# microsoft/OpenMSFTL

Measured on AMD Instinct MI355X. Metric: device-resident grad encode+decode GB/s at 1/2/4/8 MI355X; % HBM roofline, higher is better.
Workload: dtype fp32; 1 GPU; BASELINE configs[3] per-GPU shard: clients x 134,217,728-fp32 gradients, top-k f=0.1 encode -> FedAVG decode-accumulate; clients_per_gpu=128, n=134217728, codec=top, k=13421773, parallelism=dp1

## Files before the change

### openmsftl_amd/csrc/fc_capi.hip

```cpp
#include <math.h>
#include <stdarg.h>
#include <stdio.h>
#include <stdlib.h>
#include <string.h>

#include <algorithm>
#include <mutex>
#include <vector>

#include <hip/hip_ext.h>

#include "fc_state.h"

using namespace fc;

static thread_local char g_err[512];

static int fail(int code, const char* fmt, ...) {
  va_list ap;
  va_start(ap, fmt);
  vsnprintf(g_err, sizeof g_err, fmt, ap);
  va_end(ap);
  return code;
}

#define FC_CHECK(cond, ...) \
  do { if (!(cond)) return fail(FC_ERR_ARG, __VA_ARGS__); } while (0)
#define FC_LAUNCHED(name)                                                          \
  do {                                                                             \
    hipError_t e_ = hipGetLastError();                                             \
    if (e_ != hipSuccess) return fail(FC_ERR_HIP, "%s: %s", name, hipGetErrorString(e_)); \
  } while (0)

static uint32_t index_bits(uint64_t n) {
  uint32_t b = 1;
  while (b < 32 && (1ull << b) < n) ++b;
  return b;
}

static uint32_t num_chunks(uint64_t n) { return (uint32_t)((n + kChunk - 1) / kChunk); }

static WsPtrs ws_ptrs(void* ws, uint64_t n) {
  const WsLayout L = WsLayout::of(n);
  char* b = static_cast<char*>(ws);
  WsPtrs W;
  W.st = reinterpret_cast<TopkState*>(b);
  W.hist1 = reinterpret_cast<uint32_t*>(b + L.off_hist1);
  W.tick = reinterpret_cast<uint32_t*>(b + L.off_tick);
  W.ehist = reinterpret_cast<uint32_t*>(b + L.off_ehist);
  W.chist = reinterpret_cast<uint32_t*>(b + L.off_chist);
  W.small = reinterpret_cast<uint64_t*>(b + L.off_small);
  W.smallv = reinterpret_cast<uint32_t*>(b + L.off_smallv);
  W.pub = reinterpret_cast<uint32_t*>(b + L.off_pub);
  W.ccnt = reinterpret_cast<uint32_t*>(b + L.off_status);
  W.cand = reinterpret_cast<uint64_t*>(b + L.off_cand);
  W.cand_cap = L.cand_cap;
  return W;
}

static uint32_t decode_grid(uint64_t n, uint32_t per_cu = kDecBlocksPerCU) {
#ifdef FC_DEBUG_BUILD
  static const uint32_t forced = [] {
    const char* e = getenv("FC_DECODE_GRID");
    return e ? (uint32_t)atoi(e) : 0u;
  }();
#else
  constexpr uint32_t forced = 0;
#endif
  uint32_t g = forced ? forced : 256u * per_cu;
  const uint32_t nch = num_chunks(n);
  return g < nch ? g : nch;
}

constexpr int FC_MAX_SAMPLE_SEGS = 1024;
constexpr int FC_SAMPLE_DIV = 64;
constexpr int FC_SAMPLE_DIV_SINGLE = 32;
constexpr int FC_MAX_SAMPLE_SEGS_SINGLE = 2048;
constexpr int FC_SAMPLE_ROUNDS = 4;
constexpr int FC_CAND_PER_BIN = 128;
static uint32_t cand_bins_log2(uint64_t n, const SamplePlan& P) {
  if (P.full || P.lo_all || P.hi_none) return 12;
  const double S = (double)P.nseg * 1024.0;
  const double expect = (double)(P.r_lo - P.r_hi) * (double)n / S;
  uint32_t lg = 8;
  while (lg < 12 && (double)(1u << lg) * FC_CAND_PER_BIN < expect) ++lg;
  return lg;
}
static SamplePlan make_plan(uint64_t n, uint64_t k, bool single = false) {
  SamplePlan P;
  memset(&P, 0, sizeof P);
  P.n = n;
  if (n <= kFullSampleMax) {
    P.full = 1;
    P.nseg = (uint32_t)((n + 1023) / 1024);
    P.r_hi = P.r_lo = (int64_t)k;
  } else {
    uint64_t seg = n / (single ? FC_SAMPLE_DIV_SINGLE : FC_SAMPLE_DIV) / 1024;
    if (seg < 64) seg = 64;
    const uint64_t cap = single ? FC_MAX_SAMPLE_SEGS_SINGLE : FC_MAX_SAMPLE_SEGS;
    if (seg > cap) seg = cap;
    P.nseg = (uint32_t)seg;
    const double S = (double)seg * 1024.0;
    const double q = (double)k / (double)n;
    const double rho = q * S;
    const double m = 6.0 * sqrt(S * q * (1.0 - q)) + 16.0;
    P.r_hi = (int64_t)floor(rho - m);
    P.r_lo = (int64_t)ceil(rho + m);
    if (P.r_lo > (int64_t)S) P.lo_all = 1;
  }
  if (P.r_hi < 1) P.hi_none = 1;
  P.cbins_log2 = 12;
  P.segs = n <= (32ull << 20) ? 2u : (uint32_t)kSampleSegs;
  P.pstride = (P.nseg + P.segs - 1) / P.segs;
  P.np = 0;
  while (P.np < P.segs && P.np * P.pstride < P.nseg) ++P.np;
  double Sp = 0.0;
  for (uint32_t j = 0; j < P.np; ++j) {
    const uint64_t st = seg_start(P, pilot_seg(P, j));
    const uint64_t lim = P.full ? std::min<uint64_t>(st + 1024, n) : st + 1024;
    Sp += (double)(lim - st);
  }
  const double S = P.full ? (double)n : (double)P.nseg * 1024.0;
  const double q = (double)k / (double)n;
  const double sig = sqrt(Sp * q * (1.0 - q));
  const int64_t isp = (int64_t)Sp;
  P.pr_hi = std::max<int64_t>(1, (int64_t)floor((double)P.r_hi * Sp / S - 7.0 * sig - 8.0));
  P.pr_lo = std::min<int64_t>(isp, (int64_t)ceil((double)P.r_lo * Sp / S + 7.0 * sig + 8.0));
  if (P.pr_hi > isp) P.pr_hi = isp;
  if (P.pr_lo < P.pr_hi) P.pr_lo = P.pr_hi;
  return P;
}

static int check_common(const float* g, uint64_t n, void* ws, size_t ws_bytes) {
  FC_CHECK(g != nullptr, "g is NULL");
  FC_CHECK(n >= 1 && n <= 0xffffffffull, "n=%llu outside [1, 2^32-1]", (unsigned long long)n);
  FC_CHECK(((uintptr_t)g & 15) == 0, "g must be 16-byte aligned");
  FC_CHECK(ws != nullptr, "workspace is NULL");
  if (ws_bytes < WsLayout::of(n).bytes)
    return fail(FC_ERR_WORKSPACE, "workspace %zu B < %llu B needed", ws_bytes,
// ... 903 lines not shown
```

### openmsftl_amd/csrc/fc_decode.hip

```cpp
#include <type_traits>

#include "fc_state.h"

namespace fc {

struct PktCache {
  const void* idx;
  const float* val;
  const uint32_t* bitmap;
  const uint32_t* cnt;
  uint64_t thresh, seed, offset;
  double p;
  uint32_t ib, codec, key_mode;
  float w;
};

__device__ __forceinline__ PktCache load_pkt(const fc_packet_view& v) {
  PktCache c;
  c.idx = v.idx; c.val = v.val; c.bitmap = v.bitmap; c.cnt = v.cnt; c.w = v.weight;
  const fc_packet_hdr* h = v.hdr;
  c.thresh = h->thresh; c.seed = h->seed; c.offset = h->offset; c.p = h->p;
  c.ib = h->index_bits; c.codec = h->codec; c.key_mode = h->key_mode;
  return c;
}
// ... 449 lines not shown
          const float s2 = __fadd_rn(tile[loc], term);
          tile[loc] = s2;
          if (poison) cntC[loc] = (uint8_t)(cntC[loc] + 1u);
        } else {
          tile[loc] = v;
        }
      };
      if (!generic) {
        uint32_t loc[kSR];
        bool ok[kSR];
        float tv[kSR];
#pragma unroll
        for (int r = 0; r < kSR; ++r) {
          const uint32_t e = (uint32_t)(tid + r * kSBlock);
          loc[r] = ids[d][r];
          const bool keep = thresh == 0 || comp_of(mag_key(vs[d][r]), (uint32_t)base + loc[r], ib) >= thresh;
          ok[r] = e < cn[d] && keep && loc[r] < (uint32_t)kChunk;
          tv[r] = 0.f;
          if (ACC && ok[r]) tv[r] = tile[loc[r]];
        }
#pragma unroll
        for (int r = 0; r < kSR; ++r) {
          if (!ok[r]) continue;
          if (ACC) {
            const float s2 = __fadd_rn(tv[r], __fmul_rn(vs[d][r], w));
            tile[loc[r]] = s2;
            if (poison) cntC[loc[r]] = (uint8_t)(cntC[loc[r]] + 1u);
          } else {
            tile[loc[r]] = vs[d][r];
          }
        }
      } else {
        const PktCache pk = meta_pkt_s(pm);
        for (int r = 0; r < kSR; ++r) {
          const uint32_t e = (uint32_t)(tid + r * kSBlock);
          const uint32_t lc = ids[d][r];
          const float v = vs[d][r];
          if (e < cn[d] && entry_kept(pk, (uint32_t)base + lc, v)) fold(lc, scale ? (float)((double)v / pk.p) : v);
        }
      }
      if (cn[d] > (uint32_t)(kSR * kSBlock)) {
        const PktCache pk = meta_pkt_s(pm);
        gf32* pval = (gf32*)uni_ptr(pm.val) + base;
        gu16* pidx = (gu16*)uni_ptr(pm.idx) + base;
        for (uint32_t e = (uint32_t)(kSR * kSBlock + tid); e < cn[d]; e += kSBlock) {
          const uint32_t lc = pidx[e];
          const float v = pval[e];
          if (entry_kept(pk, (uint32_t)base + lc, v)) fold(lc, scale ? (float)((double)v / pk.p) : v);
        }
        __builtin_amdgcn_s_waitcnt(0x0F70);
      }
      __syncthreads();
      if (m + 1 == M) {
        write_tile(c);
        const uint32_t cnext = c + G;
        if (t + 1 < T) {
          __syncthreads();
          init_tile(cnext);
          __syncthreads();
        }
      }
    }
  };
  issue_cnt(0);
  issue_cnt(1);
  issue_ent(0);
  init_tile(blockIdx.x);
  __syncthreads();
  for (uint32_t t0 = 0; t0 < T; t0 += 2 * kSGroup) {
    issue_cnt(0);
    issue_ent(1);
    process(0, t0);
    if (t0 + kSGroup >= T) break;
    issue_cnt(1);
    issue_ent(0);
    process(1, t0 + kSGroup);
  }
}

constexpr int kQBlock = 256;
constexpr int kQuarter = kChunk / 4;
constexpr int FC_QR = 4;
constexpr int kQR = FC_QR;
constexpr int FC_QG = 3;
constexpr int kQGroup = FC_QG;
constexpr int FC_QTAIL = 8;
constexpr int kQTail = FC_QTAIL > FC_QR ? FC_QTAIL : FC_QR;

static_assert(kSparseMaxM <= 128, "k_fold_q reads the quarter offsets of <= 128 packets "
                                   "(lanes 0..63 and 64..127)");

struct QMeta {
  const void* idx;
  const float* val;
  const void* qoff;
  const fc_packet_hdr* hdr;
  uint64_t thresh;
  float w;
  uint32_t flags;
};
constexpr uint32_t kQNoQoff = 1u << 25;
constexpr uint64_t kQWhole = 1ull << 63;

template <bool DEC>
__device__ __forceinline__ void fold_q_entry(const PktCache& pk, float w, float* qt,
                                             uint32_t qbase, uint32_t id, float v) {
  if (!entry_kept(pk, id, v)) return;
  const float x = pk.codec == FC_CODEC_DROPOUT_UNBIASED ? (float)((double)v / pk.p) : v;
  const uint32_t loc = id - qbase;
  if (loc < (uint32_t)kQuarter) qt[loc] = DEC ? x : __fadd_rn(qt[loc], __fmul_rn(x, w));
}

template <bool ACC_IN, bool DEC = false>
__global__ __launch_bounds__(kQBlock, 4) void k_fold_q(DecodeArgs a) {
  __shared__ __attribute__((aligned(16))) float tile[kChunk];
  __shared__ QMeta s_meta[kSparseMaxM];
  __shared__ uint32_t s_mark[4][kQuarter / 32];
  __shared__ uint32_t s_slow;
  const int tid = threadIdx.x, lane = lane_id();
  const int q = __builtin_amdgcn_readfirstlane(tid >> 6);
  const uint32_t M = (uint32_t)a.m;
  const uint32_t c = blockIdx.x;
  const uint64_t base = (uint64_t)c * kChunk;
  const uint32_t qbase = (uint32_t)base + (uint32_t)(q * kQuarter);
  if (tid == 0) s_slow = 0;
  s_mark[q][lane] = 0u;
  __syncthreads();
  if (tid < (int)M) {
    const fc_packet_view v = DEC ? a.one : a.views[tid];
    const fc_packet_hdr* h = v.hdr;
    QMeta d;
    d.idx = v.idx; d.val = v.val; d.hdr = h;
    d.qoff = v.qoff ? (const void*)v.qoff : (const void*)v.cnt;
    d.thresh = h->thresh; d.w = v.weight;
    const uint32_t codec = h->codec, key_mode = h->key_mode;
    const float dz = (codec == FC_CODEC_DROPOUT_UNBIASED && h->p == 0.0) ? __uint_as_float(0x7fc00000u) : 0.0f;
    const bool poison = __fmul_rn(dz, v.weight) != __fmul_rn(dz, v.weight);
    const bool generic = codec == FC_CODEC_DROPOUT_UNBIASED || (key_mode == FC_KEY_PHILOX && d.thresh != 0) ||
                         (d.thresh >> (h->index_bits & 0xffu)) >= 0x7f800000ull;
    d.flags = (h->index_bits & 0xffu) | ((codec & 0xffu) << 8) | ((key_mode & 0xffu) << 16) |
              ((uint32_t)poison << 24) | (v.qoff ? 0u : kQNoQoff);
    s_meta[tid] = d;
    if (poison || generic) atomicOr(&s_slow, 1u);
  }
  __syncthreads();
  const bool slow = s_slow != 0;
  typedef __attribute__((address_space(1))) const uint64_t gu64;
  typedef __attribute__((address_space(1))) const uint32_t gu32c;
  auto qload = [&](uint32_t m) -> uint64_t {
    const QMeta& pm = s_meta[m];
    if (pm.flags & kQNoQoff) return kQWhole | ((gu32c*)pm.qoff)[c];
    return ((gu64*)pm.qoff)[c];
  };
  const uint64_t qo0 = (uint32_t)lane < M ? qload((uint32_t)lane) : 0ull;
  const uint64_t qo1 = (uint32_t)lane + 64 < M ? qload((uint32_t)lane + 64) : 0ull;
  auto qcount = [&](uint64_t v) -> uint32_t {
    if (v & kQWhole) return kQuarter + 1u;
    const uint32_t st = q == 0 ? 0u : (uint32_t)(v >> (16 * (q - 1))) & 0xffffu;
    const uint32_t en = q == 3 ? (uint32_t)(v >> 48) : (uint32_t)(v >> (16 * q)) & 0xffffu;
    return en - st;
  };
  const bool dense_q = __any(qcount(qo0) > (uint32_t)(kQTail * 64) || qcount(qo1) > (uint32_t)(kQTail * 64));
  auto range = [&](uint32_t m, uint32_t& st, uint32_t& en) {
    const uint64_t src = m < 64 ? qo0 : qo1;
    const uint32_t lo = (uint32_t)__builtin_amdgcn_readlane((int)(uint32_t)src, (int)(m & 63));
    const uint32_t hi = (uint32_t)__builtin_amdgcn_readlane((int)(uint32_t)(src >> 32), (int)(m & 63));
    const uint64_t v = ((uint64_t)hi << 32) | lo;
    st = q == 0 ? 0u : (uint32_t)(v >> (16 * (q - 1))) & 0xffffu;
    en = q == 3 ? (uint32_t)(v >> 48) : (uint32_t)(v >> (16 * q)) & 0xffffu;
    if (v & kQWhole) { st = 0u; en = lo & 0xffffu; }
  };
  float* qt = tile + q * kQuarter;
  float dz0 = 0.f;
  if (DEC) {
    const fc_packet_hdr* h = (const fc_packet_hdr*)uni_ptr(s_meta[0].hdr);
    if (h->codec == FC_CODEC_DROPOUT_UNBIASED && h->p == 0.0) dz0 = __uint_as_float(0x7fc00000u);
  }
#pragma unroll
  for (int i = 0; i < kQuarter / 256; ++i) {
    const uint32_t loc = (uint32_t)(i * 256 + lane * 4);
    float4 v = make_float4(dz0, dz0, dz0, dz0);
    if (ACC_IN) v = load4(reinterpret_cast<const float*>(a.out), (uint64_t)qbase + loc, a.n);
    *reinterpret_cast<float4*>(&qt[loc]) = v;
  }
  if (slow || dense_q) {
    for (uint32_t m = 0; m < M; ++m) {
      uint32_t st, en;
      range(m, st, en);
      const QMeta& pm = s_meta[m];
      const fc_packet_hdr* h = (const fc_packet_hdr*)uni_ptr(pm.hdr);
      PktCache pk;
      pk.thresh = uni64(pm.thresh); pk.ib = uni32(pm.flags) & 0xffu;
      pk.codec = (uni32(pm.flags) >> 8) & 0xffu; pk.key_mode = (uni32(pm.flags) >> 16) & 0xffu;
      pk.seed = h->seed; pk.offset = h->offset; pk.p = h->p;
      const float w = __uint_as_float(uni32(__float_as_uint(pm.w)));
      gu16* pidx = (gu16*)uni_ptr(pm.idx) + base;
      gf32* pval = (gf32*)uni_ptr(pm.val) + base;
      if (!DEC && ((uni32(pm.flags) >> 24) & 1u)) {
        for (uint32_t e = st + lane; e < en; e += 64) {
          const uint32_t id = (uint32_t)base + pidx[e];
          const uint32_t loc = id - qbase;
          if (loc < (uint32_t)kQuarter && entry_kept(pk, id, pval[e]))
            atomicOr(&s_mark[q][loc >> 5], 1u << (loc & 31));
        }
        const uint32_t bits = s_mark[q][lane];
        for (int b = 0; b < 32; ++b)
          if (!((bits >> b) & 1u)) qt[lane * 32 + b] = __uint_as_float(0x7fc00000u);
        s_mark[q][lane] = 0u;
      }
      for (uint32_t e = st + lane; e < en; e += 64)
        fold_q_entry<DEC>(pk, w, qt, qbase, (uint32_t)base + pidx[e], pval[e]);
    }
  } else {
    uint32_t ids_[2][kQGroup][kQR];
    float vs_[2][kQGroup][kQR];
    uint32_t qn_[2][kQGroup];
    auto issue = [&](int sl, uint32_t m0) {
#pragma unroll
      for (int d = 0; d < kQGroup; ++d) {
        const uint32_t m = min(m0 + (uint32_t)d, M - 1);
        uint32_t st, en;
        range(m, st, en);
        qn_[sl][d] = en - st;
        const QMeta& pm = s_meta[m];
        gf32* val = (gf32*)uni_ptr(pm.val) + base + st;
        gu16* idx = (gu16*)uni_ptr(pm.idx) + base + st;
        const uint32_t last = en > st ? en - st - 1u : 0u;
#pragma unroll
        for (int r = 0; r < kQR; ++r) {
          const uint32_t e = min((uint32_t)(lane + r * 64), last);
          vs_[sl][d][r] = val[e];
          ids_[sl][d][r] = idx[e];
        }
      }
    };
    auto process = [&](int sl, uint32_t m0) {
#pragma unroll
      for (int d = 0; d < kQGroup; ++d) {
        const uint32_t m = m0 + (uint32_t)d;
        if (m >= M) break;
        const QMeta& pm = s_meta[m];
        const float w = __uint_as_float(uni32(__float_as_uint(pm.w)));
        const uint64_t thresh = uni64(pm.thresh);
        const uint32_t ib = uni32(pm.flags) & 0xffu;
        const float Tf = __uint_as_float((uint32_t)(thresh >> ib));
        const uint32_t Ti = (uint32_t)(thresh & ((1ull << ib) - 1ull));
        const uint32_t b32 = (uint32_t)base;
        const uint32_t Tr = Ti <= b32 ? 0u : min(Ti - b32, (uint32_t)kChunk);
        const uint32_t qn = qn_[sl][d];
        const int lim = (int)qn - lane;
        float* slot[kQR];
        float tv[kQR];
        float* dummy = reinterpret_cast<float*>(&s_mark[q][lane]);
#pragma unroll
        for (int r = 0; r < kQR; ++r) {
          const uint32_t lc = ids_[sl][d][r];
          const float v = vs_[sl][d][r];
          const float av = __builtin_fabsf(v);
          const bool ok = (lim > r * 64) & (!(av <= Tf) | ((av == Tf) & (lc >= Tr)));
          slot[r] = ok ? qt + (lc & (uint32_t)(kQuarter - 1)) : dummy;
          tv[r] = DEC ? 0.f : *slot[r];
        }
#pragma unroll
        for (int r = 0; r < kQR; ++r)
          *slot[r] = DEC ? vs_[sl][d][r] : __fadd_rn(tv[r], __fmul_rn(vs_[sl][d][r], w));
        if (kQTail > kQR && qn > (uint32_t)(kQR * 64)) {
          uint32_t st, en;
          range(m, st, en);
          gf32* val = (gf32*)uni_ptr(pm.val) + base;
          gu16* idx = (gu16*)uni_ptr(pm.idx) + base;
          for (uint32_t e = st + (uint32_t)(kQR * 64) + lane; e < en; e += 64) {
            const uint32_t lc = idx[e];
            const float v = val[e];
            const float av = __builtin_fabsf(v);
            const uint32_t l2 = lc & (uint32_t)(kQuarter - 1);
            if (!(av <= Tf) | ((av == Tf) & (lc >= Tr)))
              qt[l2] = DEC ? v : __fadd_rn(qt[l2], __fmul_rn(v, w));
          }
        }
      }
    };
    issue(0, 0);
    for (uint32_t m0 = 0; m0 < M; m0 += 2 * kQGroup) {
      issue(1, m0 + kQGroup);
      process(0, m0);
      if (m0 + kQGroup >= M) break;
      issue(0, m0 + 2 * kQGroup);
      process(1, m0 + kQGroup);
    }
  }
  float* out = reinterpret_cast<float*>(a.out);
#pragma unroll
  for (int i = 0; i < kQuarter / 256; ++i) {
    const uint32_t loc = (uint32_t)(i * 256 + lane * 4);
    store_out(out, (uint64_t)qbase + loc, a.n, *reinterpret_cast<const float4*>(&qt[loc]));
  }
}

struct DecResArgs {
  const uint16_t* idx;
  const float* val;
  const uint64_t* qoff;
  fc_packet_hdr* hdr;
  float* out;
  uint64_t n;
  uint32_t ib, pad_;
  WsPtrs W;
};

__global__ __launch_bounds__(kQBlock, 4) void k_decode_res(DecResArgs a) {
  __shared__ __attribute__((aligned(16))) float tile[kChunk];
  __shared__ uint32_t s_skip[4][kQuarter / 32];
  __shared__ uint32_t s_fin[4];
  __shared__ uint64_t s_T;
  const int tid = threadIdx.x, lane = lane_id();
  const int q = __builtin_amdgcn_readfirstlane(tid >> 6);
  const uint32_t c = blockIdx.x;
  const uint64_t base = (uint64_t)c * kChunk;
  const uint32_t qbase = (uint32_t)base + (uint32_t)(q * kQuarter);
  const uint64_t qo = a.qoff[c];
  TopkState* S = a.W.st;
  const uint32_t t_lo = S->t_lo, t_hi = S->t_hi, sbin = S->sbin;
  const uint32_t beta = S->rb_beta, flags = S->rb_flags, cnt = S->rb_cnt;
  const bool gather = (flags & 3u) == 0;
  float* qt = tile + q * kQuarter;
#pragma unroll
  for (int i = 0; i < kQuarter / 256; ++i)
    *reinterpret_cast<float4*>(&qt[i * 256 + lane * 4]) = make_float4(0.f, 0.f, 0.f, 0.f);
  s_skip[q][lane] = 0u;
  if (lane == 0) s_fin[q] = 0u;
  __builtin_amdgcn_fence(__ATOMIC_RELEASE, "wavefront");
  __builtin_amdgcn_wave_barrier();
  bool finisher = false;
  if (!(flags & 1u)) {
    const uint32_t st = q == 0 ? 0u : (uint32_t)(qo >> (16 * (q - 1))) & 0xffffu;
    const uint32_t en = q == 3 ? (uint32_t)(qo >> 48) : (uint32_t)(qo >> (16 * q)) & 0xffffu;
    gu16* pidx = (gu16*)a.idx + base;
    gf32* pval = (gf32*)a.val + base;
    for (uint32_t e = st + (uint32_t)lane; e < en; e += 64) {
      const uint32_t lc = pidx[e];
      const float v = pval[e];
      const uint32_t key = mag_key(v);
      const uint32_t loc = lc & (uint32_t)(kQuarter - 1);
      const uint32_t bin = (key - t_lo) >> sbin;
      const bool cand = key <= t_hi;
      if (!cand || bin > beta) {
        qt[loc] = v;
      } else if (bin == beta && gather) {
        const uint32_t pos = atomicAdd(&S->small_n, 1u);
        st_agent(&a.W.small[pos], comp_of(key, (uint32_t)base + lc, a.ib));
        st_agent(&a.W.smallv[pos], __float_as_uint(v));
        atomicOr(&s_skip[q][loc >> 5], 1u << (loc & 31));
        asm volatile("s_waitcnt vmcnt(0)" ::: "memory");
        if (atomicAdd(&S->small_done, 1u) == cnt - 1u) finisher = true;
      }
    }
  }
  if (finisher) s_fin[q] = 1u;
  __builtin_amdgcn_fence(__ATOMIC_ACQ_REL, "wavefront");
  __builtin_amdgcn_wave_barrier();
  float* out = a.out;
#pragma unroll
  for (int i = 0; i < kQuarter / 256; ++i) {
    const uint32_t loc = (uint32_t)(i * 256 + lane * 4);
    const float4 v = *reinterpret_cast<const float4*>(&qt[loc]);
    const uint32_t skip = (s_skip[q][loc >> 5] >> (loc & 31)) & 0xfu;
    const uint64_t e = (uint64_t)qbase + loc;
    if (!skip) {
      store_out(out, e, a.n, v);
    } else {
      if (!(skip & 1u) && e + 0 < a.n) out[e + 0] = v.x;
// ... 129 lines not shown
```

### openmsftl_amd/csrc/fc_state.h

```cpp
#pragma once
#include <stdint.h>
#include "../../include/fedcodec.h"
#include "fc_common.h"

namespace fc {

struct alignas(16) TopkState {
  uint64_t ticket;
  uint64_t L64;
  uint64_t e_prefix;
  uint32_t err;
  uint32_t a_done, b_done, r_done;
  uint32_t pad0_[3];
  uint32_t win_flag;
  uint32_t pad1_[2];
  uint32_t t_lo, t_hi;
  uint32_t sbin;
  uint32_t cand_on, n_cand, cand_over, ent_over;
  uint32_t small_n;
  uint32_t e_shift, e_rank, e_matched, e_done, e_ticket, e_status;
  uint32_t gen;
  uint32_t small_done;
  uint32_t fz_seq;
  uint32_t hgen;
  uint32_t rb_beta, rb_rin, rb_cnt;
  uint32_t rb_flags;
  uint32_t rb_nent, rb_ncand;
  uint32_t shard_ent[kShards];
  uint32_t shard_cnd[kShards];
};
static_assert(sizeof(TopkState) <= 1024, "state block");

constexpr int FC_SAMPLE_SHARDS = 2;
constexpr int FC_CAND_SHARDS = 2;
constexpr int kSampleShards = FC_SAMPLE_SHARDS;
constexpr int kCandShards = FC_CAND_SHARDS;
constexpr int kTickGroups = 16;
constexpr int kTickStride = 64;
constexpr int kTickWords = (kTickGroups + 1) * kTickStride;
constexpr int kPubCopies = 64;
constexpr int kWinCopies = 16;
constexpr int kPubStride = 32;
constexpr int kPubWords = (kPubCopies + kWinCopies) * kPubStride;

struct WsLayout {
  uint64_t nchunks, cand_cap;
  uint64_t off_hist1, off_tick, off_ehist, off_chist, off_small, off_smallv, off_pub, off_status,
      off_cand, bytes;
  __host__ __device__ static WsLayout of(uint64_t n) {
    WsLayout L;
    L.nchunks = (n + kChunk - 1) / kChunk;
    L.cand_cap = L.nchunks * kCandSlot;
    uint64_t o = 1024;
    L.off_hist1 = o;  o += 4ull * kHistBins * kSampleShards;
    L.off_tick = o;   o += 4ull * kTickWords * 3;
    L.off_ehist = o;  o += 4ull * kHistBins;
    o += 8192;
    L.off_chist = o;  o += 4ull * kHistBins * kCandShards;
    L.off_small = o;  o += 8ull * kSmallCap;
    L.off_smallv = o; o += 4ull * kSmallCap;
    L.off_pub = o;    o += 4ull * kPubWords;
    L.off_status = o; o += 4ull * (L.nchunks ? L.nchunks : 1);
    o = (o + 15) & ~15ull;
    L.off_cand = o;   o += 8ull * L.cand_cap;
    L.bytes = (o + 255) & ~255ull;
    return L;
  }
};

struct HdrInit {
  uint64_t seed, offset;
  double p;
  uint32_t n, k, ib, codec, format, key_mode;
};

struct WsPtrs {
  TopkState* st;
  uint32_t *hist1, *tick, *ehist, *chist;
  uint64_t* small;
  uint32_t* smallv;
  uint32_t* pub;
  uint32_t* ccnt;
  uint64_t* cand;
  uint64_t cand_cap;
};

__device__ __forceinline__ WsPtrs ws_shift(WsPtrs W, uint64_t bytes) {
  W.st = reinterpret_cast<TopkState*>(reinterpret_cast<char*>(W.st) + bytes);
  W.hist1 = reinterpret_cast<uint32_t*>(reinterpret_cast<char*>(W.hist1) + bytes);
  W.tick = reinterpret_cast<uint32_t*>(reinterpret_cast<char*>(W.tick) + bytes);
  W.ehist = reinterpret_cast<uint32_t*>(reinterpret_cast<char*>(W.ehist) + bytes);
  W.chist = reinterpret_cast<uint32_t*>(reinterpret_cast<char*>(W.chist) + bytes);
  W.small = reinterpret_cast<uint64_t*>(reinterpret_cast<char*>(W.small) + bytes);
  W.smallv = reinterpret_cast<uint32_t*>(reinterpret_cast<char*>(W.smallv) + bytes);
  W.pub = reinterpret_cast<uint32_t*>(reinterpret_cast<char*>(W.pub) + bytes);
  W.ccnt = reinterpret_cast<uint32_t*>(reinterpret_cast<char*>(W.ccnt) + bytes);
  W.cand = reinterpret_cast<uint64_t*>(reinterpret_cast<char*>(W.cand) + bytes);
  return W;
}

__device__ __forceinline__ void write_hdr_static(fc_packet_hdr* h, const HdrInit& hi) {
  h->thresh = 0; h->lower = 0;
  h->n = hi.n; h->k = hi.k; h->n_entries = 0; h->index_bits = hi.ib;
  h->codec = hi.codec; h->status = FC_STATUS_OK; h->n_definite = 0; h->n_cand = 0;
  h->seed = hi.seed; h->offset = hi.offset; h->p = hi.p;
  h->chunk = kChunk; h->format = hi.format; h->key_mode = hi.key_mode;
  h->reserved[0] = h->reserved[1] = h->reserved[2] = 0;
}

struct SamplePlan {
  uint64_t n;
  uint32_t nseg;
  uint32_t full;
  int64_t r_hi, r_lo;
  uint32_t hi_none, lo_all;
  uint32_t np;
  uint32_t pstride;
  int64_t pr_hi, pr_lo;
  uint32_t cbins_log2;
  uint32_t segs;
};
constexpr int FC_SAMPLE_SEGS_PER_WG = 4;
constexpr int kPilotSegs = FC_SAMPLE_SEGS_PER_WG;
constexpr uint64_t kFullSampleMax = 1ull << 20;

__host__ __device__ __forceinline__ uint64_t seg_start(const SamplePlan& P, uint32_t s) {
  if (P.full || P.nseg == 1) return (uint64_t)s * 1024;
  return ((uint64_t)s * (P.n - 1024) / (P.nseg - 1)) & ~3ull;
}
__host__ __device__ __forceinline__ uint32_t pilot_seg(const SamplePlan& P, uint32_t j) {
  return j * P.pstride;
}

}
```

### openmsftl_amd/csrc/fc_topk.hip

```cpp
#include <type_traits>

#include "fc_state.h"

namespace fc {

template <int KM>
__device__ __forceinline__ uint4 keys4(const float4& x, uint64_t e, uint64_t seed,
                                       uint64_t off) {
  if (KM == kKeyMag) return make_uint4(mag_key(x.x), mag_key(x.y), mag_key(x.z), mag_key(x.w));
  return make_uint4(philox_word(e, seed, off) >> 1, philox_word(e + 1, seed, off) >> 1,
                    philox_word(e + 2, seed, off) >> 1, philox_word(e + 3, seed, off) >> 1);
}
template <int KM>
__device__ __forceinline__ uint32_t key1(float x, uint64_t i, uint64_t seed, uint64_t off) {
  if (KM == kKeyMag) return mag_key(x);
  return philox_word(i, seed, off) >> 1;
}
__device__ __forceinline__ uint32_t u4get(const uint4& v, int j) {
  return j == 0 ? v.x : j == 1 ? v.y : j == 2 ? v.z : v.w;
}

__device__ __forceinline__ void rank_owner(uint32_t r, uint32_t excl, uint32_t sum, uint32_t total,
                                           uint32_t* s_own) {
  if (r >= 1 && r <= total && r > excl && r <= excl + sum) { s_own[0] = threadIdx.x; s_own[1] = excl; }
// ... 860 lines not shown
  MagShared m;
};

template <bool DENSE, int NW>
__device__ __forceinline__ void fused_mag_wg(const CompactArgs& a0, const SamplePlan& P,
                                             const HdrInit& HI, uint32_t nsamp) {
  __shared__ __attribute__((aligned(16))) FusedShared u;
  __shared__ MagState s_st;
  TopkState* S = a0.W.st;
  const uint32_t pub = sload2(&S->fz_seq).x + 1u;
  if (blockIdx.x < nsamp) {
    if (threadIdx.x >= kBlock) return;
    sample_body<kKeyMag, false>(a0.g, P, 0ull, 0ull, a0.W, a0.ib, a0.hdr, HI, blockIdx.x, nsamp, false, u.s, pub);
    return;
  }
  const uint32_t chunk = blockIdx.x - nsamp;
  float x[MagGeo<NW>::kQ];
  if (chunk < 1024u) __builtin_amdgcn_s_sleep(90);
  const uint32_t* rec = &a0.W.pub[(blockIdx.x % kPubCopies) * kPubStride];
  const uint32_t tag = pub | 0x80000000u;
  typedef __attribute__((address_space(4))) const fc_rec4 fc_crec4;
  const bool try_s = !DENSE && chunk >= (uint32_t)FC_FUSED_SREC;
  fc_rec4 sr = {0u, 0u, 0u, 0u};
  if (try_s) sr = *(fc_crec4*)rec;
  mag_load<NW>(a0.g, chunk, a0.n, x);
  FC_TR(24);
  MagState st;
  if (try_s && sr.w == tag) {
    st.t_lo = sr.x; st.t_hi = sr.y; st.sbin = sr.z; st.cand_on = 1u;
    st.L64 = (uint64_t)sr.x << a0.ib;
  } else {
  if (threadIdx.x == 0) {
    uint32_t it = 0;
    fc_rec4 r = ld16_agent(rec);
    while (r.w != tag && ++it < kSpinMax) {
      __builtin_amdgcn_s_sleep(4);
      r = ld16_agent(rec);
    }
    if (it >= kSpinMax) st_agent(&S->err, 1u);
    MagState m;
    m.t_lo = r.x; m.t_hi = r.y; m.sbin = r.z; m.cand_on = 1u;
    m.L64 = (uint64_t)r.x << a0.ib;
    s_st = m;
  }
  __syncthreads();
  FC_TR(25);
  st = s_st;
  }
  compact_mag_item<NW, MagShared, DENSE, true, !DENSE>(a0, mag_out(a0, 0u), chunk, st, x, u.m);
  FC_TR(26);
}
template <bool DENSE>
__global__ __launch_bounds__(kCBlock, FC_MAG1_WAVES_PER_EU) void k_fused_mag(CompactArgs a0, SamplePlan P,
                                                                              HdrInit HI, uint32_t nsamp) {
  fused_mag_wg<DENSE, 8>(a0, P, HI, nsamp);
}
template __global__ void k_fused_mag<false>(CompactArgs, SamplePlan, HdrInit, uint32_t);
template __global__ void k_fused_mag<true>(CompactArgs, SamplePlan, HdrInit, uint32_t);

struct ResolveArgs {
  uint32_t ib, nchunks;
  uint64_t k;
  const uint16_t* idx;
  const float* val;
  const uint32_t* cnt;
  uint64_t seed, offset;
  uint32_t key_mode;
  fc_packet_hdr* hdr;
  WsPtrs W;
  const fc_encode_job* jobs;
  uint64_t ws_stride;
  float* dense;
  uint32_t rbin;
};

constexpr int kResolveChunksMax = 1024;

template <bool BIN>
__global__ __launch_bounds__(kBlock) void k_resolve(ResolveArgs a0) {
  ResolveArgs a = a0;
  apply_job(a);
  __shared__ uint64_t sv[kSmallCap];
  __shared__ uint32_t s_pre[kResolveChunksMax];
  __shared__ uint32_t s_tmp[8], s_out[4], s_flag, s_cnt, s_base, s_tot[2];
  __shared__ uint64_t s_T;
  uint32_t* h = reinterpret_cast<uint32_t*>(sv);
  TopkState* S = a.W.st;
  const int tid = threadIdx.x;
  FC_TR(8);
  uint32_t se = 0, sc = 0;
  if (tid < kShards) { se = S->shard_ent[tid]; sc = S->shard_cnd[tid]; }
  const uint32_t t_lo = S->t_lo, t_hi = S->t_hi, sbin = S->sbin, err = S->err;
  const bool rbin = a.rbin != 0;
  const uint32_t per = (a.nchunks + gridDim.x - 1) / gridDim.x;
  const uint32_t c0 = blockIdx.x * per;
  const uint32_t c1 = min(c0 + per, a.nchunks);
  const uint32_t nc = c1 > c0 ? c1 - c0 : 0u;
  const uint32_t cc_early = (nc <= (uint32_t)kBlock && (uint32_t)tid < nc) ? a.W.ccnt[c0 + tid] : 0u;
  uint32_t hv[kHistBins / kBlock];
  const bool own_hist = !BIN && !rbin;
#pragma unroll
  for (int j = 0; j < kHistBins / kBlock; ++j) hv[j] = own_hist ? a.W.chist[j * kBlock + tid] : 0u;
  static_assert(kShards == 64, "shard totals: one wave");
  if (tid < 64) {
    se = wave_sum(se);
    sc = wave_sum(sc);
    if (tid == 0) {
      s_tot[0] = se; s_tot[1] = sc;
      if (!BIN && rbin) { s_out[0] = ld_agent(&S->rb_beta); s_out[1] = ld_agent(&S->rb_rin);
                          s_out[2] = ld_agent(&S->rb_cnt); }
    }
  }
#pragma unroll
  for (int j = 0; j < kHistBins / kBlock; ++j) h[j * kBlock + tid] = hv[j];
  __syncthreads();
  const uint32_t n_ent = s_tot[0], n_cand = s_tot[1];
  const uint32_t n_hi = n_ent - n_cand;
  const bool bad = err || n_cand > n_ent || (uint64_t)n_ent < a.k || (uint64_t)n_hi > a.k;
  const uint32_t rank = bad ? 0u : (uint32_t)(a.k - n_hi);
  bool retry = bad || per > (uint32_t)kResolveChunksMax;
  uint32_t beta = 0, r_in = 1, cnt_beta = 0;
  if (!BIN && !retry && rank > 0) {
    if (own_hist) {
      find_rank_desc(h, rank, s_tmp, s_out);
      beta = s_out[0]; r_in = s_out[1]; cnt_beta = h[beta];
    } else {
      beta = s_out[0]; r_in = s_out[1]; cnt_beta = s_out[2];
    }
    retry = cnt_beta > (uint32_t)kSmallCap || cnt_beta < r_in;
    __syncthreads();
  }
  const bool binning = BIN && !retry && rank > 0;
  const bool walk = BIN ? binning : (!retry && (rank > 0 || a.dense));
  if (BIN && !binning) return;
  if (walk) {
    for (uint32_t lc = tid; lc < nc; lc += kBlock) {
      const uint32_t c = c0 + lc;
      const uint32_t cc = nc <= (uint32_t)kBlock ? cc_early : a.W.ccnt[c];
      s_pre[lc] = cc > (uint32_t)kCandSlot ? (a.cnt[c] | 0x80000000u) : cc;
    }
    __syncthreads();
  }
  FC_TR(10);
  constexpr int kGatherU = 8;
  uint32_t tpc = 64;
  while (tpc > 4 && tpc * nc > (uint32_t)kBlock) tpc >>= 1;
  uint64_t v0[kGatherU];
#pragma unroll
  for (int u = 0; u < kGatherU; ++u) v0[u] = ~0ull;
  auto for_cands = [&](bool reuse, auto&& fn) {
    const uint32_t cpr = (uint32_t)kBlock / tpc;
    for (uint32_t cb = 0; cb < nc; cb += cpr) {
      const uint32_t lc = cb + (uint32_t)tid / tpc, q = (uint32_t)tid % tpc;
      const uint32_t info = lc < nc ? s_pre[lc] : 0u;
      const uint32_t sz = info & 0x7fffffffu;
      const bool ovf = (info >> 31) != 0;
      const uint32_t c = c0 + lc;
      for (uint32_t r0 = q; r0 < sz; r0 += tpc * kGatherU) {
        const bool first = cb == 0 && r0 == q;
        uint64_t v[kGatherU];
#pragma unroll
        for (int u = 0; u < kGatherU; ++u) {
          const uint32_t r = r0 + (uint32_t)u * tpc;
          v[u] = ~0ull;
          if (reuse && first) {
            v[u] = v0[u];
          } else if (r < sz) {
            if (!ovf) {
              v[u] = a.W.cand[(uint64_t)c * kCandSlot + r];
            } else {
              const uint64_t p = (uint64_t)c * kChunk + r;
              const uint32_t id = c * (uint32_t)kChunk + a.idx[p];
              const uint32_t key = a.key_mode == FC_KEY_PHILOX ? (philox_word(id, a.seed, a.offset) >> 1)
                                                               : mag_key(a.val[p]);
              v[u] = (key >= t_lo && key <= t_hi) ? comp_of(key, id, a.ib) : ~0ull;
            }
          }
        }
        if (first && !reuse) {
#pragma unroll
          for (int u = 0; u < kGatherU; ++u) v0[u] = v[u];
        }
        fn(v);
      }
    }
  };
  auto bin_of = [&](uint64_t v) { return (((uint32_t)(v >> a.ib)) - t_lo) >> sbin; };
  if constexpr (BIN) {
    for_cands(false, [&](const uint64_t (&v)[kGatherU]) {
#pragma unroll
      for (int u = 0; u < kGatherU; ++u)
        if (v[u] != ~0ull) atomicAdd(&h[bin_of(v[u])], 1u);
    });
    __syncthreads();
    FC_TR(29);
    const uint32_t nb = min((uint32_t)kHistBins, ((t_hi - t_lo) >> sbin) + 1u);
    flush_hist(a.W.chist + (blockIdx.x % kCandShards) * kHistBins, h, nb);
    FC_TR(27);
    if (!last_block_arrive_tree(a.W.tick + 2 * kTickWords, gridDim.x, blockIdx.x, &s_flag)) return;
    constexpr int kPer = kHistBins / kBlock;
    uint32_t t[kPer];
#pragma unroll
    for (int j = 0; j < kPer; ++j) t[j] = 0;
#pragma unroll
    for (int sh = 0; sh < kCandShards; ++sh)
#pragma unroll
      for (int j = 0; j < kPer; ++j)
        if ((uint32_t)(j * kBlock + tid) < nb) t[j] += ld_agent(&a.W.chist[sh * kHistBins + j * kBlock + tid]);
#pragma unroll
    for (int j = 0; j < kPer; ++j) h[j * kBlock + tid] = t[j];
    __syncthreads();
    find_rank_desc(h, rank, s_tmp, s_out);
    if (tid == 0) {
      st_agent(&S->rb_beta, s_out[0]); st_agent(&S->rb_rin, s_out[1]);
      st_agent(&S->rb_cnt, h[s_out[0]]);
    }
    for (int sh = 0; sh < kCandShards; ++sh)
      for (uint32_t b = tid; b < nb; b += kBlock) a.W.chist[sh * kHistBins + b] = 0u;
    FC_TR(28);
    return;
  } else {
    if (!retry && rank > 0) {
      if (tid == 0) s_cnt = 0;
      __syncthreads();
      for_cands(false, [&](const uint64_t (&v)[kGatherU]) {
#pragma unroll
        for (int u = 0; u < kGatherU; ++u) {
          if (v[u] != ~0ull && bin_of(v[u]) == beta) {
            const uint32_t q = atomicAdd(&s_cnt, 1u);
            if (q < (uint32_t)kSmallCap) sv[q] = v[u];
          }
        }
      });
      __syncthreads();
      if (tid == 0 && s_cnt) s_base = atomicAdd(&S->small_n, min(s_cnt, (uint32_t)kSmallCap));
      __syncthreads();
      const uint32_t mine = min(s_cnt, (uint32_t)kSmallCap);
      for (uint32_t q = tid; q < mine; q += kBlock)
        if (s_base + q < (uint32_t)kSmallCap) st_agent(&a.W.small[s_base + q], sv[q]);
    }
    FC_TR(11);
    const uint64_t imask = (1ull << a.ib) - 1;
    if (a.dense && walk) {
      const uint32_t below = rank > 0 ? beta : 0xffffffffu;
      for_cands(rank > 0, [&](const uint64_t (&v)[kGatherU]) {
#pragma unroll
        for (int u = 0; u < kGatherU; ++u)
          if (v[u] != ~0ull && bin_of(v[u]) < below) a.dense[v[u] & imask] = 0.0f;
      });
    }
    if (!last_block_arrive_tree(a.W.tick + kTickWords, gridDim.x, blockIdx.x, &s_flag, 16)) return;
    FC_TR(12);
    uint64_t T = 0;
    uint32_t first_below = 0, list_n = 0;
    bool sorted = false;
    if (retry) {
      T = 0;
    } else if (a.k == 0) {
      T = kSelectNothing;
    } else if (rank == 0) {
      T = ((uint64_t)t_hi + 1) << a.ib;
    } else if (cnt_beta <= (uint32_t)kBlock) {
      uint64_t mine = 0;
      if ((uint32_t)tid < cnt_beta) { mine = ld_agent(&a.W.small[tid]); sv[tid] = mine; }
      __syncthreads();
      if ((uint32_t)tid < cnt_beta) {
        uint32_t larger = 0;
        for (uint32_t j = 0; j < cnt_beta; ++j) larger += sv[j] > mine ? 1u : 0u;
        if (larger == r_in - 1) s_T = mine;
      }
      __syncthreads();
      T = s_T;
      list_n = cnt_beta;
    } else {
      uint32_t P2 = 1;
      while (P2 < cnt_beta) P2 <<= 1;
      for (uint32_t i = tid; i < P2; i += kBlock) sv[i] = i < cnt_beta ? ld_agent(&a.W.small[i]) : 0ull;
      __syncthreads();
      bitonic_desc(sv, P2);
      T = sv[r_in - 1];
      first_below = r_in; list_n = cnt_beta; sorted = true;
    }
    const bool other_err = ld_agent(&S->err) != 0u;
    const uint32_t status = retry || other_err ? (uint32_t)FC_STATUS_RETRY_EXACT : (uint32_t)FC_STATUS_OK;
    FC_TR(14);
    if (a.dense && status == FC_STATUS_OK && rank > 0) {
      for (uint32_t i = (sorted ? first_below : 0u) + tid; i < list_n; i += kBlock) {
        const uint64_t v = sv[i];
        if (v < T) a.dense[v & imask] = 0.0f;
      }
    }
    if (!rbin)
      for (int b = tid; b < kHistBins; b += kBlock) a.W.chist[b] = 0;
    if (tid == 0) {
      a.hdr->thresh = T;
      a.hdr->n_entries = n_ent;
      if (status != FC_STATUS_OK) a.hdr->status = status;
      a.hdr->n_definite = n_hi;
      a.hdr->n_cand = n_cand;
      S->small_n = 0; S->err = 0;
      S->fz_seq += 1u;
    }
    FC_TR(15);
  }
}
template __global__ void k_resolve<true>(ResolveArgs);
template __global__ void k_resolve<false>(ResolveArgs);

__global__ __launch_bounds__(kBlock) void k_beta(ResolveArgs a) {
  __shared__ uint32_t h[kHistBins];
  __shared__ uint32_t s_tmp[8], s_out[4], s_tot[2];
  beta_body<false>(a.W, a.k, h, s_tmp, s_out, s_tot);
  TopkState* S = a.W.st;
  const int tid = threadIdx.x;
  for (int b = tid; b < kHistBins; b += kBlock) a.W.chist[b] = 0;
  if (tid == 0) {
    const uint32_t flags = S->rb_flags, n_ent = S->rb_nent, n_cand = S->rb_ncand;
    a.hdr->n_entries = n_ent;
    a.hdr->n_definite = n_ent - n_cand;
    a.hdr->n_cand = n_cand;
    if (flags & 1u) { a.hdr->thresh = 0; a.hdr->status = FC_STATUS_RETRY_EXACT; }
    else if (flags & 2u) a.hdr->thresh = ((uint64_t)S->t_hi + 1) << a.ib;
    S->err = 0;
    S->small_n = 0; S->small_done = 0;
    S->fz_seq += 1u;
  }
}


struct EngineArgs {
  const float* g;
  uint64_t n;
// ... 119 lines not shown
```

Measured before the change: 4307 GB/s.

## Record per-chunk bin occupancy to skip chunks in sparse resolve; deepen fold pipeline

During the binning pass, each chunk now records a 64-bit occupancy mask of which histogram bin groups its candidates hit. The sparse resolve pass uses that mask to compact the chunk list to only those chunks that can hold the target bin, which skips gathering from chunks that cannot contribute. The decode fold kernel also replaces its two-slot, three-packet-group double buffer with a six-slot ring of single-packet groups to keep more loads in flight. The cost is extra workspace, a shuffle reduction per chunk, shared-memory atomics for compaction, and more registers in the fold ring.

```diff
diff --git a/openmsftl_amd/csrc/fc_capi.hip b/openmsftl_amd/csrc/fc_capi.hip
--- a/openmsftl_amd/csrc/fc_capi.hip
+++ b/openmsftl_amd/csrc/fc_capi.hip
@@ -55,6 +55,7 @@
   W.ccnt = reinterpret_cast<uint32_t*>(b + L.off_status);
   W.cand = reinterpret_cast<uint64_t*>(b + L.off_cand);
   W.cand_cap = L.cand_cap;
+  W.occ = reinterpret_cast<uint64_t*>(b + L.off_occ);
   return W;
 }
 
diff --git a/openmsftl_amd/csrc/fc_decode.hip b/openmsftl_amd/csrc/fc_decode.hip
--- a/openmsftl_amd/csrc/fc_decode.hip
+++ b/openmsftl_amd/csrc/fc_decode.hip
@@ -555,8 +555,12 @@
 constexpr int kQuarter = kChunk / 4;
 constexpr int FC_QR = 4;
 constexpr int kQR = FC_QR;
-constexpr int FC_QG = 3;
+constexpr int FC_QG = 1;
 constexpr int kQGroup = FC_QG;
+constexpr int FC_QSLOTS = 6;
+constexpr int kQSlots = FC_QSLOTS;
+static_assert(kQSlots >= 2, "k_fold_q: one slot folds while the others load");
+static_assert(kQSlots * kQGroup * 2 * FC_QR <= 63, "k_fold_q: the ring's loads must fit vmcnt");
 constexpr int FC_QTAIL = 8;
 constexpr int kQTail = FC_QTAIL > FC_QR ? FC_QTAIL : FC_QR;
 
@@ -685,9 +689,9 @@
         fold_q_entry<DEC>(pk, w, qt, qbase, (uint32_t)base + pidx[e], pval[e]);
     }
   } else {
-    uint32_t ids_[2][kQGroup][kQR];
-    float vs_[2][kQGroup][kQR];
-    uint32_t qn_[2][kQGroup];
+    uint32_t ids_[kQSlots][kQGroup][kQR];
+    float vs_[kQSlots][kQGroup][kQR];
+    uint32_t qn_[kQSlots][kQGroup];
     auto issue = [&](int sl, uint32_t m0) {
 #pragma unroll
       for (int d = 0; d < kQGroup; ++d) {
@@ -753,13 +757,15 @@
         }
       }
     };
-    issue(0, 0);
-    for (uint32_t m0 = 0; m0 < M; m0 += 2 * kQGroup) {
-      issue(1, m0 + kQGroup);
-      process(0, m0);
-      if (m0 + kQGroup >= M) break;
-      issue(0, m0 + 2 * kQGroup);
-      process(1, m0 + kQGroup);
+#pragma unroll
+    for (int s = 0; s < kQSlots - 1; ++s) issue(s, (uint32_t)(s * kQGroup));
+    for (uint32_t m0 = 0; m0 < M; m0 += kQSlots * kQGroup) {
+#pragma unroll
+      for (int s = 0; s < kQSlots; ++s) {
+        if (s > 0 && m0 + (uint32_t)(s * kQGroup) >= M) break;
+        issue((s + kQSlots - 1) % kQSlots, m0 + (uint32_t)((s + kQSlots - 1) * kQGroup));
+        process(s, m0 + (uint32_t)(s * kQGroup));
+      }
     }
   }
   float* out = reinterpret_cast<float*>(a.out);
diff --git a/openmsftl_amd/csrc/fc_state.h b/openmsftl_amd/csrc/fc_state.h
--- a/openmsftl_amd/csrc/fc_state.h
+++ b/openmsftl_amd/csrc/fc_state.h
@@ -46,7 +46,7 @@
 struct WsLayout {
   uint64_t nchunks, cand_cap;
   uint64_t off_hist1, off_tick, off_ehist, off_chist, off_small, off_smallv, off_pub, off_status,
-      off_cand, bytes;
+      off_cand, off_occ, bytes;
   __host__ __device__ static WsLayout of(uint64_t n) {
     WsLayout L;
     L.nchunks = (n + kChunk - 1) / kChunk;
@@ -63,6 +63,7 @@
     L.off_status = o; o += 4ull * (L.nchunks ? L.nchunks : 1);
     o = (o + 15) & ~15ull;
     L.off_cand = o;   o += 8ull * L.cand_cap;
+    L.off_occ = o;    o += 8ull * (L.nchunks ? L.nchunks : 1);
     L.bytes = (o + 255) & ~255ull;
     return L;
   }
@@ -83,6 +84,7 @@
   uint32_t* ccnt;
   uint64_t* cand;
   uint64_t cand_cap;
+  uint64_t* occ;
 };
 
 __device__ __forceinline__ WsPtrs ws_shift(WsPtrs W, uint64_t bytes) {
@@ -96,6 +98,7 @@
   W.pub = reinterpret_cast<uint32_t*>(reinterpret_cast<char*>(W.pub) + bytes);
   W.ccnt = reinterpret_cast<uint32_t*>(reinterpret_cast<char*>(W.ccnt) + bytes);
   W.cand = reinterpret_cast<uint64_t*>(reinterpret_cast<char*>(W.cand) + bytes);
+  W.occ = reinterpret_cast<uint64_t*>(reinterpret_cast<char*>(W.occ) + bytes);
   return W;
 }
 
diff --git a/openmsftl_amd/csrc/fc_topk.hip b/openmsftl_amd/csrc/fc_topk.hip
--- a/openmsftl_amd/csrc/fc_topk.hip
+++ b/openmsftl_amd/csrc/fc_topk.hip
@@ -966,7 +966,7 @@
   apply_job(a);
   __shared__ uint64_t sv[kSmallCap];
   __shared__ uint32_t s_pre[kResolveChunksMax];
-  __shared__ uint32_t s_tmp[8], s_out[4], s_flag, s_cnt, s_base, s_tot[2];
+  __shared__ uint32_t s_tmp[8], s_out[4], s_flag, s_cnt, s_base, s_tot[2], s_nl;
   __shared__ uint64_t s_T;
   uint32_t* h = reinterpret_cast<uint32_t*>(sv);
   TopkState* S = a.W.st;
@@ -990,7 +990,7 @@
     se = wave_sum(se);
     sc = wave_sum(sc);
     if (tid == 0) {
-      s_tot[0] = se; s_tot[1] = sc;
+      s_tot[0] = se; s_tot[1] = sc; s_nl = 0;
       if (!BIN && rbin) { s_out[0] = ld_agent(&S->rb_beta); s_out[1] = ld_agent(&S->rb_rin);
                           s_out[2] = ld_agent(&S->rb_cnt); }
     }
@@ -1017,29 +1017,36 @@
   const bool binning = BIN && !retry && rank > 0;
   const bool walk = BIN ? binning : (!retry && (rank > 0 || a.dense));
   if (BIN && !binning) return;
+  static_assert(kResolveChunksMax <= 1024 && kChunk < (1 << 14), "s_pre word");
+  const bool sparse = !BIN && rbin && !a.dense && walk;
+  uint32_t nl = nc;
   if (walk) {
     for (uint32_t lc = tid; lc < nc; lc += kBlock) {
       const uint32_t c = c0 + lc;
+      const uint64_t occ = sparse ? a.W.occ[c] : ~0ull;
       const uint32_t cc = nc <= (uint32_t)kBlock ? cc_early : a.W.ccnt[c];
-      s_pre[lc] = cc > (uint32_t)kCandSlot ? (a.cnt[c] | 0x80000000u) : cc;
+      const uint32_t word = (cc > (uint32_t)kCandSlot ? (a.cnt[c] | 0x80000000u) : cc) | (lc << 14);
+      if (!sparse) s_pre[lc] = word;
+      else if ((occ >> (beta >> 6)) & 1ull) s_pre[atomicAdd(&s_nl, 1u)] = word;
     }
     __syncthreads();
+    if (sparse) nl = s_nl;
   }
   FC_TR(10);
   constexpr int kGatherU = 8;
   uint32_t tpc = 64;
-  while (tpc > 4 && tpc * nc > (uint32_t)kBlock) tpc >>= 1;
+  while (tpc > 4 && tpc * nl > (uint32_t)kBlock) tpc >>= 1;
   uint64_t v0[kGatherU];
 #pragma unroll
   for (int u = 0; u < kGatherU; ++u) v0[u] = ~0ull;
-  auto for_cands = [&](bool reuse, auto&& fn) {
+  auto for_cands = [&](bool reuse, auto&& fn, auto&& done) {
     const uint32_t cpr = (uint32_t)kBlock / tpc;
-    for (uint32_t cb = 0; cb < nc; cb += cpr) {
-      const uint32_t lc = cb + (uint32_t)tid / tpc, q = (uint32_t)tid % tpc;
-      const uint32_t info = lc < nc ? s_pre[lc] : 0u;
-      const uint32_t sz = info & 0x7fffffffu;
+    for (uint32_t cb = 0; cb < nl; cb += cpr) {
+      const uint32_t li = cb + (uint32_t)tid / tpc, q = (uint32_t)tid % tpc;
+      const uint32_t info = li < nl ? s_pre[li] : 0u;
+      const uint32_t sz = info & 0x3fffu;
       const bool ovf = (info >> 31) != 0;
-      const uint32_t c = c0 + lc;
+      const uint32_t c = c0 + ((info >> 14) & 0x3ffu);
       for (uint32_t r0 = q; r0 < sz; r0 += tpc * kGatherU) {
         const bool first = cb == 0 && r0 == q;
         uint64_t v[kGatherU];
@@ -1067,14 +1074,25 @@
         }
         fn(v);
       }
+      if (li < nl) done(c, q);
     }
   };
+  auto no_done = [](uint32_t, uint32_t) {};
   auto bin_of = [&](uint64_t v) { return (((uint32_t)(v >> a.ib)) - t_lo) >> sbin; };
   if constexpr (BIN) {
+    uint64_t occ = 0;
     for_cands(false, [&](const uint64_t (&v)[kGatherU]) {
 #pragma unroll
       for (int u = 0; u < kGatherU; ++u)
-        if (v[u] != ~0ull) atomicAdd(&h[bin_of(v[u])], 1u);
+        if (v[u] != ~0ull) {
+          const uint32_t b = bin_of(v[u]);
+          atomicAdd(&h[b], 1u);
+          occ |= 1ull << (b >> 6);
+        }
+    }, [&](uint32_t c, uint32_t q) {
+      for (uint32_t m = tpc >> 1; m; m >>= 1) occ |= __shfl_xor(occ, (int)m);
+      if (q == 0) a.W.occ[c] = occ;
+      occ = 0;
     });
     __syncthreads();
     FC_TR(29);
@@ -1115,7 +1133,7 @@
             if (q < (uint32_t)kSmallCap) sv[q] = v[u];
           }
         }
-      });
+      }, no_done);
       __syncthreads();
       if (tid == 0 && s_cnt) s_base = atomicAdd(&S->small_n, min(s_cnt, (uint32_t)kSmallCap));
       __syncthreads();
@@ -1131,7 +1149,7 @@
 #pragma unroll
         for (int u = 0; u < kGatherU; ++u)
           if (v[u] != ~0ull && bin_of(v[u]) < below) a.dense[v[u] & imask] = 0.0f;
-      });
+      }, no_done);
     }
     if (!last_block_arrive_tree(a.W.tick + kTickWords, gridDim.x, blockIdx.x, &s_flag, 16)) return;
     FC_TR(12);
```

Result: no change. 4306 GB/s (-0.0%).
